# Cogito2012/OpenTAL

Measured on AMD Instinct MI355X. Metric: clips/sec training step, 256-frame THUMOS14 clips, higher is better.
Workload: dtype bf16

## Files before the change

### include/opental_hip.h

```cpp
#ifndef OPENTAL_HIP_H
#define OPENTAL_HIP_H

#include <stdint.h>
#include <stddef.h>

#ifdef __cplusplus
extern "C" {
#endif

#define OTAL_ABI_VERSION 26

#define OTAL_E_NULL      (-1)
#define OTAL_E_SHAPE     (-2)
#define OTAL_E_ODD_C     (-3)
#define OTAL_E_BATCH     (-4)
#define OTAL_E_DTYPE     (-5)
#define OTAL_E_LEVELS    (-6)
#define OTAL_E_UNSUPPORTED (-7)

#define OTAL_F32  0
#define OTAL_BF16 1
#define OTAL_F16  2
#define OTAL_F64  3

// ... 43 lines not shown
                         float* const* dw, int precision, void* ws, size_t ws_bytes, void* stream);

size_t otal_conv_prologue_bytes(const int* geom, const int64_t* strides, int mode, int precision);
size_t otal_conv_prologue_desc_bytes(void);
int otal_conv_prologue(const int* geom, const int64_t* strides, int mode, const float* w, int precision, void* region,
                       size_t region_bytes, void* host_desc, void* stream);
int otal_conv_prologue_batch(int n, const void* device_descs, const int* device_starts, int total_blocks, void* stream);

int otal_conv_defer_reduces(int on);
size_t otal_conv_deferred_end(void);
int otal_conv_deferred_count(void);
int otal_conv_flush_reduces(void* stream);

const char* otal_conv_last_kernel(void);

int otal_conv_pack_wt(const float* w, float* wt, int Cout, int Cin, int kvol, void* stream);

int otal_gn_relu_fwd(const float* x, const float* gamma, const float* beta, float* y, float* stats,
                     int B, int C, int T, int G, float eps, int relu, int nlev, const int* lev, void* stream);
int otal_gn_relu_bwd(const float* dy, int64_t dy_batch_stride, const float* x, const float* gamma, const float* beta,
                     const float* stats, float* dx, float* partial, int B, int C, int T, int G,
                     int relu, int nlev, const int* lev, void* stream);
int otal_gn_relu_fwd_pair(const float* const* x, const float* const* gamma, const float* const* beta, float* const* y,
                          float* const* stats, int B, int C, int T, int G, float eps, int relu, int nlev, const int* lev,
                          void* stream);
int otal_gn_relu_bwd_pair(const float* const* dy, const int64_t* dy_batch_stride, const float* const* x,
                          const float* const* gamma, const float* const* beta, const float* const* stats, float* const* dx,
                          float* const* partial, int B, int C, int T, int G, int relu, int nlev, const int* lev, void* stream);
int otal_sum_partials(int n_items, const float* const* partial, float* const* dst0, float* const* dst1,
                      float* const* dst2, const int* channels, const int* batches, void* stream);

const char* otal_layer_last_kernel(void);

int otal_maxpool3d_fwd(const int* geom, const int64_t* strides, const float* x, float* y,
                       unsigned char* argtap, void* stream);
int otal_maxpool3d_bwd(const int* geom, const int64_t* strides, const float* dy,
                       const unsigned char* argtap, float* dx, int accumulate,
                       const float* out_mask, const float* out_scale, void* stream);
size_t otal_maxpool3d_signbits_bytes(const int* geom, const int64_t* strides);
int otal_maxpool3d_fwd_signbits(const int* geom, const int64_t* strides, const float* x, float* y,
                                unsigned char* argtap, unsigned char* signbits, void* stream);
int otal_maxpool3d_bwd_signbits(const int* geom, const int64_t* strides, const float* dy, const unsigned char* argtap,
                                float* dx, int accumulate, const unsigned char* signbits, const float* out_scale,
                                void* stream);
int otal_maxpool3d_fwd_signbits_h(const int* geom, const int64_t* strides, const void* x_bf16, float* y,
                                  unsigned char* argtap, unsigned char* signbits, void* stream);
int otal_maxpool3d_bwd_signbits_h(const int* geom, const int64_t* strides, const float* dy, const unsigned char* argtap,
                                  void* dx_bf16, const unsigned char* signbits, const float* out_scale, void* stream);
int otal_maxpool3d_fwd_io(const int* geom, const int64_t* strides, const void* x, void* y, unsigned char* argtap,
                          unsigned char* signbits, int io, void* stream);
int otal_maxpool3d_bwd_io(const int* geom, const int64_t* strides, const void* dy, const unsigned char* argtap, void* dx,
                          int accumulate, const void* out_mask, const float* out_scale, const unsigned char* signbits, int io,
                          void* stream);
int otal_convert_storage(const void* src, int64_t src_bs, int64_t src_cs, void* dst, int64_t dst_bs, int64_t dst_cs,
                         int to_bf16, int B, int C, int P, void* stream);

int otal_head_outputs_fwd(int n_items, const int* channels, const int* modes, const float* const* raw, float* const* out,
                          float* const* unct, const float* scales, int B, int N, int nlev, const int* lev,
                          const float* level_strides, void* stream);
int otal_head_outputs_bwd(int n_items, const int* channels, const int* modes, const float* const* raw,
                          const float* const* out, const float* const* unct, const float* const* dout,
                          const float* const* dunct, float* const* draw, const float* scales, float* dscales, int B,
                          int N, int nlev, const int* lev, const float* level_strides, void* stream);

int otal_boundary_bce(const float* x, int64_t x_batch_stride, int64_t x_channel_stride, const float* mask,
                      int64_t mask_batch_stride, int64_t mask_row_stride, int mask_row0, int mask_step, float* terms,
                      float* dx, int B, int C, int T, void* stream);

int otal_boundary_finish(int n, const float* const* terms, const float* weights, const int* T, int B, float* out2, void* stream);
int otal_boundary_scale(int n, const float* const* dx, float* const* out, const float* weights, const int* C, const int* T,
                        int B, const float* g_start, const float* g_end, void* stream);

int otal_proposal_windows(const float* loc, float* seg, float* frame_seg, int B, int nlev,
                          const int* lev, float frame_num, void* stream);

int otal_decode_clips(const float* loc, const float* prop_loc, const float* priors, const float* conf,
                      const float* prop_conf, const float* center, const float* act, const float* prop_act,
                      const float* offsets, const float* fps, float* seg, float* score, float* unct,
                      float* actn, unsigned char* flag, int nclips, int A, int K, float clip_length,
                      float conf_thresh, void* stream);
int otal_decode_clips_ex(const float* loc, const float* prop_loc, const float* priors, const float* conf,
                         const float* prop_conf, const float* center, const float* act, const float* prop_act,
                         const float* offsets, const float* fps, float* seg, float* score, float* unct,
                         float* actn, unsigned char* flag, int nclips, int A, int K, float clip_length,
                         float conf_thresh, int score_fn, int first_class, void* stream);
int otal_softnms_classes(const float* seg, const float* score, const float* unct, const float* actn,
                         const unsigned char* flag, const int* clip_start, int nvideos, int max_clips,
                         int A, int K, float sigma, int top_k, float score_threshold, float* out,
                         int* counts, int* out_index, int out_cols, void* stream);
size_t otal_softnms_scratch_bytes(int total_clips, int max_clips, int A, int K);
int otal_softnms_classes_ws(const float* seg, const float* score, const float* unct, const float* actn,
                            const unsigned char* flag, const int* clip_start, int nvideos, int max_clips,
                            int A, int K, float sigma, int top_k, float score_threshold, float* out,
                            int* counts, int* out_index, int out_cols, void* scratch, size_t scratch_bytes,
                            int total_clips, void* stream);
int otal_detection_table(const float* rows, const int* counts, const double* durations, int V, int K, int top_k, int cols,
                         int drop_empty, int scoring, int* video, int* cls, double* seg, float* sup, double* known,
                         int* list_start, void* stream);

int otal_openmax_dist(const float* feat, int N, int rows_per_batch, int64_t sb, int64_t sr, int64_t sc, const float* mav,
                      int K, int D, const int* labels, float* dist, void* stream);
int otal_openmax_class_means(const float* feat, int N, int rows_per_batch, int64_t sb, int64_t sr, int64_t sc,
                             const int* labels, int K, int D, float* means, int* counts, void* stream);
int otal_openmax_probs(const float* logits, int64_t ldl, const float* feat, int N, int rows_per_batch, int64_t sb, int64_t sr,
                       int64_t sc, const float* mav, const float* wb, int K, int D, int R, float* probs, void* stream);
int otal_decode_clips_openmax(const float* loc, const float* prop_loc, const float* priors, const float* conf,
// ... 106 lines not shown
```

### opental_amd/common/i3d_backbone.py

```python
import torch
import torch.nn as nn
import torch.nn.functional as F
from torch.autograd import Function

from . import ops
from .layers import MaxPool3dSamePadding

ONE, THREE = (1, 1, 1), (3, 3, 3)
BN_EPS = 1e-3


class Unit3D(nn.Module):

    def __init__(self, in_channels, output_channels, kernel_shape=(1, 1, 1), stride=(1, 1, 1), padding=0,
                 activation_fn=F.relu, use_batch_norm=True, use_bias=False, padding_valid_spatial=False,
                 name='unit_3d'):
        super(Unit3D, self).__init__()
        if not use_batch_norm or use_bias or activation_fn is not F.relu or padding_valid_spatial or padding == -1:
            raise NotImplementedError("backbone Unit3D is conv(no bias) + BN + ReLU with SAME padding")
        self._output_channels = output_channels
        self._kernel_shape = tuple(kernel_shape)
        self._stride = tuple(stride)
        self.name = name
        self.conv3d = nn.Conv3d(in_channels, output_channels, self._kernel_shape, self._stride, padding=0, bias=False)
# ... 189 lines not shown
def _fused_affine(scale, shift, offs, w0):
    key = (scale.data_ptr(), shift.data_ptr(), scale._version, w0)
    hit = _FUSED_AFFINE.get(key)
    if hit is None:
        pick = lambda t, i: t[offs[i]:offs[i + 1]]
        hit = (torch.cat([pick(scale, w0 + 1), pick(scale, w0 + 3), pick(scale, w0)]),
               torch.cat([pick(shift, w0 + 1), pick(shift, w0 + 3), pick(shift, w0)]), scale, shift)
        if len(_FUSED_AFFINE) > 256:
            _FUSED_AFFINE.clear()
        _FUSED_AFFINE[key] = hit
    return hit[0], hit[1]


_HALF_OK = {}


def _pool_half_ok(shape, k, s):
    _, _, T, H, W = shape
    k, s = tuple(k), tuple(s)
    out_positions = -(-T // s[0]) * -(-H // s[1]) * -(-W // s[2])
    if out_positions % 8:
        return False
    if k[1:] == (3, 3) and s[1:] == (2, 2) and H % 2 == 0 and W % 4 == 0:
        return (k[0], s[0]) == (1, 1) or ((k[0], s[0]) == (3, 2) and T % 2 == 0)
    return k == THREE and s == ONE and H == W and H in (12, 6)


def _conv_half_ok(shape, cout, k, first=False):
    modes = (0, 2) if first else (0, 1, 2)
    return all(ops.half_storage_ok(m, tuple(shape), cout, k, ONE, both=True) for m in modes)


def _step_half_ok(step, shape, weights):
    key = (step[0], tuple(shape), step[1:-1] if step[0] != "conv" else (tuple(weights[step[1]].shape), step[2], step[3]), ops.HALF_CHAIN,
           int(ops.CONV_PRECISION), ops.HALF_STORAGE)
    hit = _HALF_OK.get(key)
    if hit is None:
        B, C, T, H, W = shape
        if not (ops.HALF_CHAIN and ops.HALF_STORAGE and int(ops.CONV_PRECISION) & 1):
            hit = False
        elif step[0] == "conv":
            hit = tuple(step[3]) == ONE and _conv_half_ok(shape, weights[step[1]].shape[0], tuple(step[2]))
        elif step[0] == "pool":
            hit = _pool_half_ok(shape, step[1], step[2])
        else:
            oc = step[2]
            hit = (_conv_half_ok(shape, oc[1] + oc[3] + oc[0], ONE) and _conv_half_ok((B, oc[1], T, H, W), oc[2], THREE)
                   and _conv_half_ok((B, oc[3], T, H, W), oc[4], THREE) and _pool_half_ok(shape, THREE, ONE)
                   and _conv_half_ok(shape, oc[5], ONE))
        if len(_HALF_OK) > 512:
            _HALF_OK.clear()
        _HALF_OK[key] = hit
    return hit


class I3DFeaturesFunction(Function):

    @staticmethod
    def forward(ctx, x, plan, endpoints, scale, shift, offs, *weights):
        x = x.contiguous()
        sc = lambda i: scale[offs[i]:offs[i + 1]]
        sh = lambda i: shift[offs[i]:offs[i + 1]]
        tape, found, half_grads = [], {}, {}
        cur = x
        cur_scale = None
        BF = torch.bfloat16
        need_grad = any(ctx.needs_input_grad)
        raw_out = {e[1:] for e in endpoints if e.startswith("=")}
        endpoints = tuple(e.lstrip("=") for e in endpoints)

        def leave_half():
            nonlocal cur
            cur32 = ops.convert_storage(cur, torch.float32)
            tape.append(("cvt", cur, cur32, cur_scale))
            cur = cur32

        for si, step in enumerate(plan):
            kind, name = step[0], step[-1]
            chain = cur.dtype == BF and _step_half_ok(step, cur.shape, weights)
            pool_io1 = (cur.dtype == BF and not chain and kind == "pool" and cur_scale is not None
                        and tuple(step[1]) == (1, 3, 3) and tuple(step[2]) == (1, 2, 2)
                        and cur.shape[3] % 2 == 0 and cur.shape[4] % 4 == 0)
            if cur.dtype == BF and not chain and not pool_io1:
                leave_half()
            if kind == "conv" and chain:
                _, wi, k, s, _ = step
                y = ops.conv_forward(cur, weights[wi], k, s, scale=sc(wi), shift=sh(wi), relu=True)
                tape.append(("conv", wi, k, s, cur, y, cur_scale, sc(wi)))
                cur, cur_scale = y, sc(wi)
            elif kind == "conv":
                _, wi, k, s, _ = step
                pooled_next = (name not in endpoints and si + 1 < len(plan) and plan[si + 1][0] == "pool"
                               and tuple(plan[si + 1][1]) == (1, 3, 3) and tuple(plan[si + 1][2]) == (1, 2, 2)
                               and ops.half_storage_ok(0, tuple(cur.shape), weights[wi].shape[0], k, s))
                grad_half = (pooled_next and si == 0 and not x.requires_grad
                             and ops.half_storage_ok(2, tuple(cur.shape), weights[wi].shape[0], k, s))
                half = pooled_next and (grad_half or (si > 0 and ops.HALF_ACT_DIRECT))
                if (not half and si == 0 and not x.requires_grad and ops.HALF_CHAIN and si + 1 < len(plan) and name not in endpoints
                        and ops.half_storage_ok(0, tuple(cur.shape), weights[wi].shape[0], k, s)
                        and ops.half_storage_ok(2, tuple(cur.shape), weights[wi].shape[0], k, s)):
                    half = True
                half_grads[si + 1] = grad_half
                y = ops.conv_forward(cur, weights[wi], k, s, scale=sc(wi), shift=sh(wi), relu=True, half_out=half)
                tape.append(("conv", wi, k, s, cur, y, cur_scale, sc(wi)))
                cur, cur_scale = y, sc(wi)
            elif kind == "pool":
# ... 38 lines not shown
                    ops.conv_forward(pm, weights[w0 + 5], ONE, ONE, scale=sc(w0 + 5), shift=sh(w0 + 5), relu=True,
                                     out=Y[:, c3:])
                out_scale = _cat_cached(_OUT_SCALE, scale, w0, [sc(w0), sc(w0 + 2), sc(w0 + 4), sc(w0 + 5)])
                tape.append(("mixed", w0, (c1, c2, c3), cur, h1, h2, pm, argm, Y, cur_scale, (wf, o1, o13), out_scale))
                cur, cur_scale = Y, out_scale
            if name in endpoints:
                if cur.dtype == BF and name not in raw_out:
                    ends = si + 1 == len(plan) or not _step_half_ok(plan[si + 1], cur.shape, weights)
                    if need_grad or ends:
                        leave_half()
                        found[name] = (cur, len(tape))
                    else:
                        found[name] = (ops.convert_storage(cur, torch.float32), len(tape))
                else:
                    found[name] = (cur, len(tape))
                hooks = ops.STEP.endpoint_hooks
                hook = hooks.get(name) if hooks else None
                if hook is not None:
                    hook(found[name][0])
        missing = [e for e in endpoints if e not in found]
        if missing:
            raise RuntimeError(f"unknown endpoints {missing}")
        ctx.tape = tape
        ctx.meta = (scale, offs, [found[e][1] for e in endpoints], len(weights), x.requires_grad)
        ctx.weights = weights
        ctx.outs = [found[e][0] for e in endpoints]
        return tuple(ctx.outs)

    @staticmethod
    def backward(ctx, *douts):
        tape, weights = ctx.tape, ctx.weights
        scale, offs, out_pos, nw, need_dx = ctx.meta
        sc = lambda i: scale[offs[i]:offs[i + 1]]
        dws = [None] * nw
        pending = {}
        for pos, g, z in zip(out_pos, douts, ctx.outs):
            if g is not None:
                pending.setdefault(pos, []).append((g, z, tape[pos - 1][-1]))
        zg = {}

        def out_grad_buffer(p, shape, like):
            if p >= 1 and tape[p - 1][0] == "mixed":
                o13 = tape[p - 1][10][2]
                B, ct, T, H, W = shape
                buf = torch.empty((B, o13 + ct, T, H, W), dtype=like.dtype, device=like.device)
                zg[p] = buf
                return buf[:, o13:]
            return torch.empty(tuple(shape), dtype=like.dtype, device=like.device)

        side = ops.side_wgrads(weights[0].device)
        in_slots = True
        dcur = None
        cloned = True
        mixed_pos = [p for p in range(1, len(tape) + 1) if tape[p - 1][0] == "mixed"]
        tail_below = min(mixed_pos) if mixed_pos and not need_dx else 0
        for pos in range(len(tape), 0, -1):
            if pos == tail_below - 1 and not any(pending.get(q) for q in range(1, pos + 1)):
                ops.late_mark([weights[st[1]] for st in tape[:pos] if st[0] == "conv"])
            for g, z, zs in pending.pop(pos, ()):
                ops.join_pending(g)
                dense = g.dim() == 5 and (g.shape[4] == 1 or g.stride(4) == 1) and (g.shape[3] == 1 or g.stride(3) == g.shape[4])
                if zs is not None and not dense:
                    g = g.contiguous()
                if dcur is None:
                    if zs is not None:
                        dcur = out_grad_buffer(pos, g.shape, g)
                        ops.masked_scale_copy(g, z, zs, dcur)
                    elif tape[pos - 1][0] == "mixed":
                        dcur = out_grad_buffer(pos, g.shape, g)
                        dcur.copy_(g)
                    else:
                        dcur = g.contiguous()
                        cloned = False
                elif zs is not None:
                    ops.masked_scale_copy(g, z, zs, dcur, accumulate=True)
                else:
                    if not cloned:
                        dcur, cloned = dcur.clone(), True
                    dcur.add_(g)
            if dcur is None:
                continue
            step = tape[pos - 1]
            first = pos == 1
            if step[0] == "cvt":
                _, xh, _, _ = step
                dcur = ops.convert_storage(dcur.contiguous(), xh.dtype, out=out_grad_buffer(pos - 1, xh.shape, xh))
            elif step[0] == "conv":
                _, wi, k, s, xin, y, in_scale, _ = step
                slot = ops.grad_slot(weights[wi])
                in_slots = in_slots and slot is not None
                if first and not need_dx:
                    side.issue()
                    dws[wi] = ops.conv_wgrad(xin, dcur, weights[wi].shape, k, s, out=slot)
                else:
                    dws[wi] = side.wgrad(xin, dcur, weights[wi].shape, k, s, out=slot)
                if first and not need_dx:
                    dcur = None
                else:
                    dcur = ops.conv_dgrad(dcur, weights[wi], xin.shape, k, s, out=out_grad_buffer(pos - 1, xin.shape, xin),
                                          out_mask=xin if in_scale is not None else None, out_scale=in_scale)
                side.flush()
                ops.grads_ready([(weights[wi], dws[wi])])
            elif step[0] == "pool":
                _, k, s, xin, (arg, bits, grad_half), in_scale, _ = step
                if dcur.dtype == torch.bfloat16:
                    masked = in_scale is not None and bits is not None
                    dcur = ops.maxpool3d_backward(dcur, arg, xin.shape, k, s, out=out_grad_buffer(pos - 1, xin.shape, xin),
                                                  out_scale=in_scale if masked else None, out_signbits=bits if masked else None)
                elif grad_half:
                    dcur = ops.maxpool3d_backward(dcur, arg, xin.shape, k, s, out_scale=in_scale, out_signbits=bits, half_out=True)
                else:
                    dcur = ops.maxpool3d_backward(dcur, arg, xin.shape, k, s, out=out_grad_buffer(pos - 1, xin.shape, dcur),
                                                  out_mask=xin if (in_scale is not None and bits is None) else None,
                                                  out_scale=in_scale, out_signbits=bits)
            else:
                _, w0, (c1, c2, c3), xin, h1, h2, pm, argm, Y, in_scale, (wf, o1, o13), _ = step
                Zg = zg.pop(pos)
                dY = Zg[:, o13:]
                dX = out_grad_buffer(pos - 1, xin.shape, xin)
                xm = xin if in_scale is not None else None
                sl = (slice(0, c1), slice(c1, c2), slice(c2, c3), slice(c3, Y.shape[1]))
                for a, b, hid, sli, dst in ((w0 + 1, w0 + 2, h1, sl[1], Zg[:, :o1]), (w0 + 3, w0 + 4, h2, sl[2], Zg[:, o1:o13])):
                    g = dY[:, sli]
                    slot = ops.grad_slot(weights[b])
                    in_slots = in_slots and slot is not None
                    dws[b] = side.wgrad(hid, g, weights[b].shape, THREE, ONE, out=slot)
                    ops.conv_dgrad(g, weights[b], hid.shape, THREE, ONE, out=dst, out_mask=hid, out_scale=sc(a))
                gf = Zg[:, :o13 + c1]
                slot = ops.grad_slot(wf)
                in_slots = in_slots and slot is not None
                dwf = side.wgrad(xin, gf, wf.shape, ONE, ONE, out=slot)
                dws[w0 + 1], dws[w0 + 3], dws[w0] = dwf[:o1], dwf[o1:o13], dwf[o13:]
                ops.conv_dgrad(gf, wf, xin.shape, ONE, ONE, out=dX, out_mask=xm, out_scale=in_scale)
                g3 = dY[:, sl[3]]
                slot = ops.grad_slot(weights[w0 + 5])
                in_slots = in_slots and slot is not None
                dws[w0 + 5] = side.wgrad(pm, g3, weights[w0 + 5].shape, ONE, ONE, out=slot)
                dpm = ops.conv_dgrad(g3, weights[w0 + 5], pm.shape, ONE, ONE)
                ops.maxpool3d_backward(dpm, argm, xin.shape, THREE, ONE, out=dX, accumulate=True,
                                       out_mask=xm, out_scale=in_scale)
                dcur = dX
                side.flush()
                ops.grads_ready([(weights[w0 + q], dws[w0 + q]) for q in range(6)])
        side.node_end(in_slots)
        ctx.tape = None
        ctx.outs = None
        dx = dcur if need_dx else None
        return (dx, None, None, None, None, None) + tuple(dws)
```

### opental_amd/common/ops.py

```python
import bisect
import ctypes
import os
import warnings

import torch

from .. import _lib as L
from .conv_geom import make_geom

_WORKSPACE = {}
WORKSPACE_BYTES = 192 << 20
WORKSPACE_TOTAL = 512 << 20

CONV_PROFILE = None

CONV_PRECISION = 0
HALF_STORAGE = os.environ.get("OTAL_HALF_STORAGE", "1") != "0"
HALF_ACT_DIRECT = os.environ.get("OTAL_HALF_ACT_DIRECT", "0") != "0"
HALF_CHAIN = os.environ.get("OTAL_HALF_CHAIN", "1") != "0"


def _prof_begin():
    if CONV_PROFILE is None:
        return None
    ev = torch.cuda.Event(enable_timing=True)
    ev.record()
    return ev


def _prof_end(ev, mode, g, problems=1):
    if ev is None:
        return
    end = torch.cuda.Event(enable_timing=True)
    end.record()
    B, Cin, Cout = g[0], g[1], g[2]
    flops = 2.0 * B * Cout * g[6] * g[7] * g[8] * Cin * g[9] * g[10] * g[11] * problems
    CONV_PROFILE.append((mode, flops, ev, end))


def workspace(device, side=False):
    key = (device.type, device.index, side)
    ws = _WORKSPACE.get(key)
    if ws is None:
        ws = torch.empty(WORKSPACE_TOTAL, dtype=torch.uint8, device=device)
        _WORKSPACE[key] = ws
    return ws


class StepState:
    def __init__(self):
        self.lanes = None
        self.slots = None
        self.ready = None
        self.defer_join = False
        self.pending_sums = None
        self.prologues = None
        self.late_weights = None
        self.endpoint_hooks = None
        self.early_results = {}
        self.pending_joins = {}
        self.defer = False
        self.defer_owner = None
        self.ws_cursor = [0, 0, 0, 0]
        self.ws_index = 0
        self.stream = None

    def begin_backward(self, slots, ready, early):
        if self.slots is not None:
            raise RuntimeError("a trainer's backward is already running in this process (one at a time)")
        self.slots, self.ready = slots, ready
        self.defer_join = early
        self.pending_sums = [] if early else None
# ... 1053 lines not shown
def maxpool3d_backward(dy, arg, x_shape, k, s, out=None, accumulate=False, out_mask=None, out_scale=None, out_signbits=None,
                       half_out=False):
    if dy.dtype == torch.bfloat16:
        if out is None:
            if accumulate:
                raise RuntimeError("accumulate needs an existing buffer")
            out = torch.empty(tuple(x_shape), dtype=torch.bfloat16, device=dy.device)
        g, outn = _pool_geom(out, k, s)
        _check(out, "dx", torch.bfloat16); _check(dy, "dy", torch.bfloat16)
        if tuple(dy.shape[2:]) != outn or not arg.is_contiguous():
            raise RuntimeError("maxpool3d_backward: shape mismatch")
        if out_mask is not None and (tuple(out_mask.shape) != tuple(out.shape) or out_mask.stride() != out.stride()
                                     or out_mask.dtype != torch.bfloat16):
            raise RuntimeError("out_mask must share dx's shape, layout and dtype")
        ga, sa = _geom_arrays(g, out, dy)
        L.check(L.lib().otal_maxpool3d_bwd_io(ga, sa, L.ptr(dy), L.ptr(arg), L.ptr(out), int(accumulate), _opt(out_mask),
                                              _opt(out_scale), _opt(out_signbits), 3 | (4 if out_mask is not None else 0), L.stream()),
                "otal_maxpool3d_bwd_io")
        return out
    if half_out:
        if accumulate or out_mask is not None or out_signbits is None or out is not None:
            raise RuntimeError("maxpool3d_backward(half_out): plain store with the sign-bit mask only")
        out = torch.empty(tuple(x_shape), dtype=torch.bfloat16, device=dy.device)
        g, outn = _pool_geom(out, k, s)
        _check(out, "dx", torch.bfloat16); _check(dy, "dy")
        if tuple(dy.shape[2:]) != outn or not arg.is_contiguous():
            raise RuntimeError("maxpool3d_backward: shape mismatch")
        ga, sa = _geom_arrays(g, out, dy)
        L.check(L.lib().otal_maxpool3d_bwd_signbits_h(ga, sa, L.ptr(dy), L.ptr(arg), L.ptr(out), L.ptr(out_signbits),
                                                      L.ptr(out_scale), L.stream()), "otal_maxpool3d_bwd_signbits_h")
        return out
    if out is None:
        if accumulate:
            raise RuntimeError("accumulate needs an existing buffer")
        out = torch.empty(tuple(x_shape), dtype=dy.dtype, device=dy.device)
    g, outn = _pool_geom(out, k, s)
    _check(out, "dx"); _check(dy, "dy")
    if tuple(dy.shape[2:]) != outn or not arg.is_contiguous():
        raise RuntimeError("maxpool3d_backward: shape mismatch")
    ga, sa = _geom_arrays(g, out, dy)
    if out_signbits is not None:
        if out.data_ptr() % 16 or dy.data_ptr() % 8:
            raise RuntimeError("maxpool3d_backward: the sign-bit path needs 16-byte aligned dx")
        L.check(L.lib().otal_maxpool3d_bwd_signbits(ga, sa, L.ptr(dy), L.ptr(arg), L.ptr(out), int(accumulate), L.ptr(out_signbits),
                                                    L.ptr(out_scale), L.stream()), "otal_maxpool3d_bwd_signbits")
        return out
    if out_mask is not None and (tuple(out_mask.shape) != tuple(out.shape) or out_mask.stride() != out.stride()):
        raise RuntimeError("out_mask must share dx's shape and layout")
    L.check(L.lib().otal_maxpool3d_bwd(ga, sa, L.ptr(dy), L.ptr(arg), L.ptr(out), int(accumulate),
                                       _opt(out_mask), _opt(out_scale), L.stream()), "otal_maxpool3d_bwd")
    return out


def convert_storage(src, dtype, out=None):
    s5 = _as5(src)
    if out is None:
        out = torch.empty(tuple(src.shape), dtype=dtype, device=src.device)
    o5 = _as5(out)
    if {src.dtype, out.dtype} != {torch.float32, torch.bfloat16} or tuple(o5.shape) != tuple(s5.shape):
        raise RuntimeError("convert_storage: float32 <-> bfloat16, same shape")
    _check(s5, "src", s5.dtype); _check(o5, "dst", o5.dtype)
    B, C, T, H, W = s5.shape
    if (T * H * W) % 8:
        out.copy_(src)
        return out
    (sb, sc), (db, dc) = _bs(s5), _bs(o5)
    L.check(L.lib().otal_convert_storage(L.ptr(s5), ctypes.c_int64(sb), ctypes.c_int64(sc), L.ptr(o5), ctypes.c_int64(db),
                                         ctypes.c_int64(dc), int(out.dtype == torch.bfloat16), B, C, T * H * W, L.stream()),
            "otal_convert_storage")
    return out


def proposal_windows(loc, levels, frame_num):
    L.require_device(loc)
    B, N, _ = loc.shape
    assert N == levels[-1]
    seg = torch.empty((B, N, 4), dtype=torch.float32, device=loc.device)
    fseg = torch.empty_like(seg)
    L.check(L.lib().otal_proposal_windows(L.ptr(loc), L.ptr(seg), L.ptr(fseg), B, len(levels) - 1,
                                          L.int_array(list(levels)), ctypes.c_float(frame_num), L.stream()),
            "otal_proposal_windows")
    return seg, fseg


def adam_flat(p, g, m, v, step, lr, beta1=0.9, beta2=0.999, eps=1e-8, weight_decay=0.0, grad_scale=1.0):
    L.require_device(p, g, m, v)
    L.check(L.lib().otal_adam_flat(L.ptr(p), L.ptr(g), L.ptr(m), L.ptr(v), ctypes.c_int64(p.numel()),
                                   ctypes.c_float(lr), ctypes.c_float(beta1), ctypes.c_float(beta2),
                                   ctypes.c_float(eps), ctypes.c_float(weight_decay), int(step),
                                   ctypes.c_float(grad_scale), L.stream()), "otal_adam_flat")


def adam_bias_corrections(step, beta1=0.9, beta2=0.999):
    import math
    import numpy as np
    b1, b2 = float(np.float32(beta1)), float(np.float32(beta2))
    return [float(np.float32(1.0 - math.pow(b1, step))), float(np.float32(math.sqrt(1.0 - math.pow(b2, step))))]


def adam_flat_dev(p, g, m, v, bias_corr, lr, beta1=0.9, beta2=0.999, eps=1e-8, weight_decay=0.0, grad_scale=1.0):
    L.require_device(p, g, m, v, bias_corr)
    L.check(L.lib().otal_adam_flat_dev(L.ptr(p), L.ptr(g), L.ptr(m), L.ptr(v), ctypes.c_int64(p.numel()),
                                       ctypes.c_float(lr), ctypes.c_float(beta1), ctypes.c_float(beta2),
                                       ctypes.c_float(eps), ctypes.c_float(weight_decay), L.ptr(bias_corr),
                                       ctypes.c_float(grad_scale), L.stream()), "otal_adam_flat_dev")

# ... 490 lines not shown
```

### opental_amd/csrc/pool3d.hip

```cpp
#include "common.h"
#include <cstdlib>

#include "pool_select.h"

namespace {

template <int KT, int KH, int KW, int ST, int SH, int SW>
struct PoolShape {
    __device__ __forceinline__ static int kt(const PoolGeom& g) { return KT ? KT : g.kt; }
    __device__ __forceinline__ static int kh(const PoolGeom& g) { return KT ? KH : g.kh; }
    __device__ __forceinline__ static int kw(const PoolGeom& g) { return KT ? KW : g.kw; }
    __device__ __forceinline__ static int st(const PoolGeom& g) { return KT ? ST : g.st; }
    __device__ __forceinline__ static int sh(const PoolGeom& g) { return KT ? SH : g.sh; }
    __device__ __forceinline__ static int sw(const PoolGeom& g) { return KT ? SW : g.sw; }
    static constexpr int UT = KT ? KT : 1, UH = KT ? KH : 1, UW = KT ? KW : 1;
    static constexpr int UCT = KT ? (KT + ST - 1) / ST : 1, UCH = KT ? (KH + SH - 1) / SH : 1, UCW = KT ? (KW + SW - 1) / SW : 1;
};

__device__ __forceinline__ float h2f_lo(unsigned w) { return __uint_as_float(w << 16); }
__device__ __forceinline__ float h2f_hi(unsigned w) { return __uint_as_float(w & 0xffff0000u); }
__device__ __forceinline__ unsigned f2h_pair_exact(float lo, float hi) {
    return (__float_as_uint(lo) >> 16) | (__float_as_uint(hi) & 0xffff0000u);
}
__device__ __forceinline__ unsigned f2h_pair_rne(float lo, float hi) {
// ... 192 lines not shown
    const int bc = blockIdx.y;
    const int b = bc / g.C, c = bc - b * g.C;
    const int to0 = blockIdx.x * TT;
    const int tt = min(TT, g.To - to0);
    const int TL = (tt - 1) * st + kt;
    const int PL = g.HL * g.WL;
    const float* xb = x + (int64_t)b * g.x_bs + (int64_t)c * g.x_cs;
    const int ti0 = to0 * st - g.pt;
    for (int i = threadIdx.x; i < TL * PL; i += 256) {
        const uint32_t tl = fd_div(g.fPL, (uint32_t)i);
        const uint32_t r = i - tl * PL;
        const uint32_t hl = fd_div(g.fWL, r);
        const int wl = (int)(r - hl * g.WL);
        const int ti = ti0 + (int)tl, hi = (int)hl - g.ph, wi = wl - g.pw;
        const bool in = (unsigned)ti < (unsigned)g.Ti && (unsigned)hi < (unsigned)g.Hi && (unsigned)wi < (unsigned)g.Wi;
        const int64_t off = in ? ((int64_t)ti * g.Hi + hi) * g.Wi + wi : 0;
        const float v = xb[off];
        sm[i] = in ? v : 0.f;
    }
    __syncthreads();
    const int Po = g.Ho * g.Wo;
    const int P = g.To * Po;
    for (int i = threadIdx.x; i < tt * Po; i += 256) {
        const uint32_t tq = fd_div(g.fPo, (uint32_t)i);
        const uint32_t r = i - tq * Po;
        const uint32_t ho = fd_div(g.fWo, r);
        const int wo = (int)(r - ho * g.Wo);
        const float* base = sm + ((int)tq * st * g.HL + (int)ho * sh) * g.WL + wo * sw;
        float best = 0.f;
        int win = 0;
        bool first = true;
#pragma unroll S::UT
        for (int dt = 0; dt < kt; ++dt)
#pragma unroll S::UH
            for (int dh = 0; dh < kh; ++dh)
#pragma unroll S::UW
                for (int dw = 0; dw < kw; ++dw) {
                    const float v = base[(dt * g.HL + dh) * g.WL + dw];
                    if (first || v > best || v != v) {
                        best = v;
                        win = (dt * kh + dh) * kw + dw;
                        first = false;
                    }
                }
        const int wdt = win / (kh * kw), wr = win - wdt * (kh * kw), wdh = wr / kw, wdw = wr - wdh * kw;
        const int ti = (to0 + (int)tq) * st - g.pt + wdt, hi = (int)ho * sh - g.ph + wdh, wi = wo * sw - g.pw + wdw;
        const bool in = (unsigned)ti < (unsigned)g.Ti && (unsigned)hi < (unsigned)g.Hi && (unsigned)wi < (unsigned)g.Wi;
        const int p = to0 * Po + i;
        y[(int64_t)b * g.y_bs + (int64_t)c * g.y_cs + p] = best;
        arg[(int64_t)bc * P + p] = (unsigned char)(in ? win : 255);
    }
}

template <int KT, int KH, int KW, int ST, int SH, int SW>
__global__ __launch_bounds__(256) void maxpool3d_bwd_lds_kernel(const float* __restrict__ dy,
                                                                const unsigned char* __restrict__ arg,
                                                                float* __restrict__ dx, PoolGeom g, int accumulate,
                                                                const float* __restrict__ emask,
                                                                const float* __restrict__ escale, int TI, int TLo_max) {
    using S = PoolShape<KT, KH, KW, ST, SH, SW>;
    extern __shared__ float sm[];
    const int kt = S::kt(g), kh = S::kh(g), kw = S::kw(g);
    const int st = S::st(g), sh = S::sh(g), sw = S::sw(g);
    constexpr int CT = KT ? (KT + ST - 1) / ST : 0, CH = KT ? (KH + SH - 1) / SH : 0, CW = KT ? (KW + SW - 1) / SW : 0;
    const int ct = KT ? CT : (kt + st - 1) / st, ch = KT ? CH : (kh + sh - 1) / sh, cw = KT ? CW : (kw + sw - 1) / sw;
    const int bc = blockIdx.y;
    const int b = bc / g.C, c = bc - b * g.C;
    const int ti0 = blockIdx.x * TI;
    const int tin = min(TI, g.Ti - ti0);
    const int toA = (ti0 + g.pt) / st - (ct - 1);
    const int toB = (ti0 + tin - 1 + g.pt) / st;
    const int TLo = toB - toA + 1;
    const int PLo = g.HLo * g.WLo;
    unsigned char* sa = reinterpret_cast<unsigned char*>(sm + TLo_max * PLo);
    const int Po = g.Ho * g.Wo;
    const float* dyb = dy + (int64_t)b * g.y_bs + (int64_t)c * g.y_cs;
    const unsigned char* ab = arg + (int64_t)bc * g.To * Po;
    for (int i = threadIdx.x; i < TLo * PLo; i += 256) {
        const uint32_t tl = fd_div(g.fPLo, (uint32_t)i);
        const uint32_t r = i - tl * PLo;
        const uint32_t hl = fd_div(g.fWLo, r);
        const int wl = (int)(r - hl * g.WLo);
        const int to = toA + (int)tl, ho = (int)hl + g.ho_min, wo = wl + g.wo_min;
        const bool in = (unsigned)to < (unsigned)g.To && (unsigned)ho < (unsigned)g.Ho && (unsigned)wo < (unsigned)g.Wo;
        const int o = in ? (to * g.Ho + ho) * g.Wo + wo : 0;
        const float d = dyb[o];
        const unsigned char a = ab[o];
        sm[i] = in ? d : 0.f;
        sa[i] = a;
    }
    __syncthreads();
    const int Pi = g.Hi * g.Wi;
    for (int i = threadIdx.x; i < tin * Pi; i += 256) {
        const uint32_t tq = fd_div(g.fPi, (uint32_t)i);
        const uint32_t r = i - tq * Pi;
        const uint32_t hi = fd_div(g.fWi, r);
        const int wi = (int)(r - hi * g.Wi);
        const int tn = ti0 + (int)tq + g.pt, hn = (int)hi + g.ph, wn = wi + g.pw;
        const int to0 = tn / st, ho0 = hn / sh, wo0 = wn / sw;
        float acc = 0.f;
#pragma unroll S::UCT
        for (int a_ = 0; a_ < ct; ++a_) {
            const int to = to0 - a_, dt = tn - to * st;
#pragma unroll S::UCH
            for (int b_ = 0; b_ < ch; ++b_) {
                const int ho = ho0 - b_, dh = hn - ho * sh;
#pragma unroll S::UCW
                for (int c_ = 0; c_ < cw; ++c_) {
                    const int wo = wo0 - c_, dw = wn - wo * sw;
                    const int idx = ((to - toA) * g.HLo + (ho - g.ho_min)) * g.WLo + (wo - g.wo_min);
                    const bool ok = dt < kt && dh < kh && dw < kw;
                    const float d = sm[idx];
                    const int a = sa[idx];
                    acc += (ok && a == (dt * kh + dh) * kw + dw) ? d : 0.f;
                }
            }
        }
        const int p = ti0 * Pi + i;
        const int64_t off = (int64_t)b * g.x_bs + (int64_t)c * g.x_cs + p;
        if (emask) acc = emask[off] > 0.f ? acc * escale[c] : 0.f;
        dx[off] = accumulate ? dx[off] + acc : acc;
    }
}

__device__ __forceinline__ void first_max3(float a, float b, float c, float& v, int& k) {
    v = a; k = 0;
    if (b > v || b != b) { v = b; k = 1; }
    if (c > v || c != c) { v = c; k = 2; }
}

template <int P>
__global__ __launch_bounds__(256) void maxpool333_sep_fwd_kernel(const float* __restrict__ x, float* __restrict__ y,
                                                                 unsigned char* __restrict__ arg, PoolGeom g, int TT, int vec) {
    extern __shared__ float sm[];
    constexpr int Q = P + 2, PL = Q * Q, PP = P * P, CR = Q * P;
    const int tid = threadIdx.x;
    const int bc = blockIdx.y;
    const int b = bc / g.C, c = bc - b * g.C;
    const int to0 = blockIdx.x * TT;
    const int tt = min(TT, g.To - to0);
    const int TL = tt + 2;
    float* xs = sm;
    float* rm = sm + (TT + 2) * PL;
    unsigned char* tw = reinterpret_cast<unsigned char*>(rm + (TT + 2) * CR);
    unsigned char* th = tw + (TT + 2) * CR;
    const float* xb = x + (int64_t)b * g.x_bs + (int64_t)c * g.x_cs;
    constexpr int VW = P % 4 == 0 ? 4 : (P % 2 == 0 ? 2 : 1);
    if (VW > 1 && vec) {
        for (int i = tid; i < TL * PL; i += 256) xs[i] = 0.f;
        __syncthreads();
        constexpr int NQ = P / VW;
        for (int i = tid; i < TL * P * NQ; i += 256) {
            const int tl = i / (P * NQ), r = i - tl * (P * NQ), hi = r / NQ, q = r - hi * NQ;
            const int ti = to0 - 1 + tl;
            if ((unsigned)ti >= (unsigned)g.Ti) continue;
            float* dst = xs + (tl * Q + hi + 1) * Q + q * VW + 1;
            if constexpr (VW == 4) {
                const float4 v = *reinterpret_cast<const float4*>(xb + (ti * P + hi) * P + q * 4);
                dst[0] = v.x; dst[1] = v.y; dst[2] = v.z; dst[3] = v.w;
            } else {
                const float2 v = *reinterpret_cast<const float2*>(xb + (ti * P + hi) * P + q * 2);
                dst[0] = v.x; dst[1] = v.y;
            }
        }
    } else {
        for (int i = tid; i < TL * PL; i += 256) {
            const int tl = i / PL, r = i - tl * PL, hl = r / Q, wl = r - hl * Q;
            const int ti = to0 - 1 + tl, hi = hl - 1, wi = wl - 1;
            const bool in = (unsigned)ti < (unsigned)g.Ti && (unsigned)hi < (unsigned)P && (unsigned)wi < (unsigned)P;
            const float v = xb[in ? (ti * P + hi) * P + wi : 0];
            xs[i] = in ? v : 0.f;
        }
    }
    __syncthreads();
// ... 875 lines not shown
        case PK_BWD_222: hipLaunchKernelGGL((maxpool3d_bwd_kernel<2, 2, 2, 2, 2, 2>), grid, block, c.lds, st_, dy, argtap, dx, g, acc, mask, scale); break;
        case PK_BWD_ANY: hipLaunchKernelGGL((maxpool3d_bwd_kernel<0, 0, 0, 0, 0, 0>), grid, block, c.lds, st_, dy, argtap, dx, g, acc, mask, scale); break;
        case PK_BWD_LDS_133: hipLaunchKernelGGL((maxpool3d_bwd_lds_kernel<1, 3, 3, 1, 2, 2>), grid, block, c.lds, st_, dy, argtap, dx, g, acc, mask, scale, c.planes, c.tlo_max); break;
        case PK_BWD_LDS_333S1: hipLaunchKernelGGL((maxpool3d_bwd_lds_kernel<3, 3, 3, 1, 1, 1>), grid, block, c.lds, st_, dy, argtap, dx, g, acc, mask, scale, c.planes, c.tlo_max); break;
        case PK_BWD_LDS_333S2: hipLaunchKernelGGL((maxpool3d_bwd_lds_kernel<3, 3, 3, 2, 2, 2>), grid, block, c.lds, st_, dy, argtap, dx, g, acc, mask, scale, c.planes, c.tlo_max); break;
        case PK_BWD_LDS_222: hipLaunchKernelGGL((maxpool3d_bwd_lds_kernel<2, 2, 2, 2, 2, 2>), grid, block, c.lds, st_, dy, argtap, dx, g, acc, mask, scale, c.planes, c.tlo_max); break;
        case PK_BWD_LDS_ANY: hipLaunchKernelGGL((maxpool3d_bwd_lds_kernel<0, 0, 0, 0, 0, 0>), grid, block, c.lds, st_, dy, argtap, dx, g, acc, mask, scale, c.planes, c.tlo_max); break;
        default: return OTAL_E_UNSUPPORTED;
    }
    return otal_layer_launched(pool_kernel_name(c.kernel));
}

extern "C" int otal_maxpool3d_fwd(const int* geom, const int64_t* strides, const float* x, float* y,
                                  unsigned char* argtap, void* stream) {
    return pool_fwd(geom, strides, x, y, argtap, nullptr, stream);
}
extern "C" int otal_maxpool3d_bwd(const int* geom, const int64_t* strides, const float* dy,
                                  const unsigned char* argtap, float* dx, int accumulate,
                                  const float* out_mask, const float* out_scale, void* stream) {
    return pool_bwd(geom, strides, dy, argtap, dx, accumulate, out_mask, out_scale, nullptr, stream);
}
extern "C" size_t otal_maxpool3d_signbits_bytes(const int* geom, const int64_t* strides) {
    if (!geom || !strides) return 0;
    PoolGeom g;
    if (fill(g, geom, strides)) return 0;
    if (!strided_k33_kind(g)) return 0;
    return (size_t)g.B * g.C * g.Ti * (g.Hi / 2) * (g.Wi / 4);
}
extern "C" int otal_maxpool3d_fwd_signbits(const int* geom, const int64_t* strides, const float* x, float* y,
                                           unsigned char* argtap, unsigned char* signbits, void* stream) {
    g_layer_kernel = "";
    if (!signbits) return OTAL_E_NULL;
    return pool_fwd(geom, strides, x, y, argtap, signbits, stream);
}
extern "C" int otal_maxpool3d_bwd_signbits(const int* geom, const int64_t* strides, const float* dy, const unsigned char* argtap,
                                           float* dx, int accumulate, const unsigned char* signbits, const float* out_scale,
                                           void* stream) {
    g_layer_kernel = "";
    if (!signbits || !out_scale) return OTAL_E_NULL;
    return pool_bwd(geom, strides, dy, argtap, dx, accumulate, nullptr, out_scale, signbits, stream);
}
extern "C" int otal_maxpool3d_fwd_signbits_h(const int* geom, const int64_t* strides, const void* x_bf16, float* y,
                                             unsigned char* argtap, unsigned char* signbits, void* stream) {
    g_layer_kernel = "";
    if (!signbits) return OTAL_E_NULL;
    return pool_fwd(geom, strides, static_cast<const float*>(x_bf16), y, argtap, signbits, stream, 1);
}
extern "C" int otal_maxpool3d_bwd_signbits_h(const int* geom, const int64_t* strides, const float* dy, const unsigned char* argtap,
                                             void* dx_bf16, const unsigned char* signbits, const float* out_scale, void* stream) {
    g_layer_kernel = "";
    if (!signbits || !out_scale) return OTAL_E_NULL;
    return pool_bwd(geom, strides, dy, argtap, static_cast<float*>(dx_bf16), 0, nullptr, out_scale, signbits, stream, 1);
}
extern "C" int otal_maxpool3d_fwd_io(const int* geom, const int64_t* strides, const void* x, void* y, unsigned char* argtap,
                                     unsigned char* signbits, int io, void* stream) {
    return pool_fwd(geom, strides, static_cast<const float*>(x), static_cast<float*>(y), argtap, signbits, stream, io);
}
extern "C" int otal_maxpool3d_bwd_io(const int* geom, const int64_t* strides, const void* dy, const unsigned char* argtap, void* dx,
                                     int accumulate, const void* out_mask, const float* out_scale, const unsigned char* signbits,
                                     int io, void* stream) {
    return pool_bwd(geom, strides, static_cast<const float*>(dy), argtap, static_cast<float*>(dx), accumulate,
                    static_cast<const float*>(out_mask), out_scale, signbits, stream, io);
}
```

Before: 1018.

## Fuse maxpool backward with bf16 convert, masked scale and residual add at seam

Adds a fused kernel for the backward pass at a pool step that directly follows an fp32-to-bf16 convert. It does the pool gradient gather, applies the ReLU mask and BN scale to both the pool gradient and a pending gradient, adds them, and writes bf16 straight into the upstream gradient buffer. The separate fp32 pool backward, the pending-gradient accumulation and the convert kernel are skipped. This removes several full-tensor fp32 read/write passes and kernel launches, in exchange for a narrower applicability check and fallbacks when the layout does not fit.

```diff
diff --git a/include/opental_hip.h b/include/opental_hip.h
--- a/include/opental_hip.h
+++ b/include/opental_hip.h
@@ -119,6 +119,9 @@
 int otal_maxpool3d_bwd_io(const int* geom, const int64_t* strides, const void* dy, const unsigned char* argtap, void* dx,
                           int accumulate, const void* out_mask, const float* out_scale, const unsigned char* signbits, int io,
                           void* stream);
+int otal_maxpool3d_bwd_seam(const int* geom, const int64_t* strides, const float* dy, const unsigned char* argtap,
+                            const void* mask_bf16, const int64_t* mask_strides, const float* out_scale,
+                            const float* add_src, const int64_t* add_strides, void* dx_bf16, void* stream);
 int otal_convert_storage(const void* src, int64_t src_bs, int64_t src_cs, void* dst, int64_t dst_bs, int64_t dst_cs,
                          int to_bf16, int B, int C, int P, void* stream);
 
diff --git a/opental_amd/common/i3d_backbone.py b/opental_amd/common/i3d_backbone.py
--- a/opental_amd/common/i3d_backbone.py
+++ b/opental_amd/common/i3d_backbone.py
@@ -265,6 +265,27 @@
             _HALF_OK.clear()
         _HALF_OK[key] = hit
     return hit
+
+
+def pool_seam_gradient(tape, pos, pending, zg, dcur):
+    if not ops.POOL_SEAM or pos < 2 or tape[pos - 1][0] != "pool" or tape[pos - 2][0] != "cvt":
+        return None
+    _, _, _, xin, (_, bits, grad_half), in_scale, _ = tape[pos - 1]
+    _, xh, x32, seam_scale = tape[pos - 2]
+    if xin is not x32 or in_scale is None or seam_scale is not in_scale or bits is not None or grad_half:
+        return None
+    if xh.dtype != torch.bfloat16 or dcur is None or dcur.dtype != torch.float32 or (pos - 2) in zg:
+        return None
+    waiting = pending.get(pos - 1) or ()
+    if len(waiting) != 1:
+        return None
+    g, z, zs = waiting[0]
+    if z is not x32 or zs is not in_scale or g.dtype != torch.float32 or g.dim() != 5 or tuple(g.shape) != tuple(xh.shape):
+        return None
+    dense = (g.shape[4] == 1 or g.stride(4) == 1) and (g.shape[3] == 1 or g.stride(3) == g.shape[4])
+    if not dense or (xh.shape[2] * xh.shape[3] * xh.shape[4]) % 8:
+        return None
+    return waiting[0]
 
 
 class I3DFeaturesFunction(Function):
@@ -409,6 +430,7 @@
         in_slots = True
         dcur = None
         cloned = True
+        seam_done = 0
         mixed_pos = [p for p in range(1, len(tape) + 1) if tape[p - 1][0] == "mixed"]
         tail_below = min(mixed_pos) if mixed_pos and not need_dx else 0
         for pos in range(len(tape), 0, -1):
@@ -439,7 +461,9 @@
                 continue
             step = tape[pos - 1]
             first = pos == 1
-            if step[0] == "cvt":
+            if step[0] == "cvt" and seam_done == pos:
+                pass
+            elif step[0] == "cvt":
                 _, xh, _, _ = step
                 dcur = ops.convert_storage(dcur.contiguous(), xh.dtype, out=out_grad_buffer(pos - 1, xh.shape, xh))
             elif step[0] == "conv":
@@ -460,6 +484,16 @@
                 ops.grads_ready([(weights[wi], dws[wi])])
             elif step[0] == "pool":
                 _, k, s, xin, (arg, bits, grad_half), in_scale, _ = step
+                seam = pool_seam_gradient(tape, pos, pending, zg, dcur)
+                if seam is not None:
+                    xh = tape[pos - 2][1]
+                    ops.join_pending(seam[0])
+                    dseam = out_grad_buffer(pos - 2, xh.shape, xh)
+                    if ops.maxpool3d_backward_seam(dcur, arg, k, s, xh, in_scale, seam[0], dseam):
+                        pending.pop(pos - 1)
+                        dcur, seam_done = dseam, pos - 1
+                        continue
+                    zg.pop(pos - 2, None)
                 if dcur.dtype == torch.bfloat16:
                     masked = in_scale is not None and bits is not None
                     dcur = ops.maxpool3d_backward(dcur, arg, xin.shape, k, s, out=out_grad_buffer(pos - 1, xin.shape, xin),
diff --git a/opental_amd/common/ops.py b/opental_amd/common/ops.py
--- a/opental_amd/common/ops.py
+++ b/opental_amd/common/ops.py
@@ -18,6 +18,7 @@
 HALF_STORAGE = os.environ.get("OTAL_HALF_STORAGE", "1") != "0"
 HALF_ACT_DIRECT = os.environ.get("OTAL_HALF_ACT_DIRECT", "0") != "0"
 HALF_CHAIN = os.environ.get("OTAL_HALF_CHAIN", "1") != "0"
+POOL_SEAM = True
 
 
 def _prof_begin():
@@ -1177,6 +1178,26 @@
     return out
 
 
+def maxpool3d_backward_seam(dy, arg, k, s, mask, scale, add_src, out):
+    B, C, T, H, W = out.shape
+    g, outn = _pool_geom(out, k, s)
+    _check(out, "dx", torch.bfloat16); _check(mask, "mask", torch.bfloat16); _check(dy, "dy")
+    if tuple(dy.shape) != (B, C) + outn or not arg.is_contiguous() or tuple(mask.shape) != tuple(out.shape):
+        raise RuntimeError("maxpool3d_backward_seam: shape mismatch")
+    if (not add_src.is_cuda or add_src.dtype != torch.float32 or tuple(add_src.shape) != tuple(out.shape)
+            or (W > 1 and add_src.stride(4) != 1) or (H > 1 and add_src.stride(3) != W)):
+        raise RuntimeError(f"maxpool3d_backward_seam: add_src must be a float32 GPU tensor of shape {tuple(out.shape)} with dense "
+                           f"H x W planes (strides {add_src.stride()})")
+    ga, sa = _geom_arrays(g, out, dy)
+    rc = L.lib().otal_maxpool3d_bwd_seam(ga, sa, L.ptr(dy), L.ptr(arg), L.ptr(mask), (ctypes.c_int64 * 2)(*_bs(mask)), L.ptr(scale),
+                                         L.ptr(add_src), (ctypes.c_int64 * 3)(add_src.stride(0), add_src.stride(1), add_src.stride(2)),
+                                         L.ptr(out), L.stream())
+    if rc == L.E_UNSUPPORTED:
+        return False
+    L.check(rc, "otal_maxpool3d_bwd_seam")
+    return True
+
+
 def convert_storage(src, dtype, out=None):
     s5 = _as5(src)
     if out is None:
diff --git a/opental_amd/csrc/pool3d.hip b/opental_amd/csrc/pool3d.hip
--- a/opental_amd/csrc/pool3d.hip
+++ b/opental_amd/csrc/pool3d.hip
@@ -268,6 +268,50 @@
     }
 }
 
+__device__ __forceinline__ void bwd_lds_stage(const float* __restrict__ dyb, const unsigned char* __restrict__ ab, const PoolGeom& g,
+                                              float* sm, unsigned char* sa, int toA, int TLo) {
+    const int PLo = g.HLo * g.WLo;
+    for (int i = threadIdx.x; i < TLo * PLo; i += 256) {
+        const uint32_t tl = fd_div(g.fPLo, (uint32_t)i);
+        const uint32_t r = i - tl * PLo;
+        const uint32_t hl = fd_div(g.fWLo, r);
+        const int wl = (int)(r - hl * g.WLo);
+        const int to = toA + (int)tl, ho = (int)hl + g.ho_min, wo = wl + g.wo_min;
+        const bool in = (unsigned)to < (unsigned)g.To && (unsigned)ho < (unsigned)g.Ho && (unsigned)wo < (unsigned)g.Wo;
+        const int o = in ? (to * g.Ho + ho) * g.Wo + wo : 0;
+        const float d = dyb[o];
+        const unsigned char a = ab[o];
+        sm[i] = in ? d : 0.f;
+        sa[i] = a;
+    }
+}
+template <class S>
+__device__ __forceinline__ float bwd_lds_gather(const float* sm, const unsigned char* sa, const PoolGeom& g, int toA, int tn, int hn, int wn,
+                                                int ct, int ch, int cw) {
+    const int kt = S::kt(g), kh = S::kh(g), kw = S::kw(g);
+    const int st = S::st(g), sh = S::sh(g), sw = S::sw(g);
+    const int to0 = tn / st, ho0 = hn / sh, wo0 = wn / sw;
+    float acc = 0.f;
+#pragma unroll S::UCT
+    for (int a_ = 0; a_ < ct; ++a_) {
+        const int to = to0 - a_, dt = tn - to * st;
+#pragma unroll S::UCH
+        for (int b_ = 0; b_ < ch; ++b_) {
+            const int ho = ho0 - b_, dh = hn - ho * sh;
+#pragma unroll S::UCW
+            for (int c_ = 0; c_ < cw; ++c_) {
+                const int wo = wo0 - c_, dw = wn - wo * sw;
+                const int idx = ((to - toA) * g.HLo + (ho - g.ho_min)) * g.WLo + (wo - g.wo_min);
+                const bool ok = dt < kt && dh < kh && dw < kw;
+                const float d = sm[idx];
+                const int a = sa[idx];
+                acc += (ok && a == (dt * kh + dh) * kw + dw) ? d : 0.f;
+            }
+        }
+    }
+    return acc;
+}
+
 template <int KT, int KH, int KW, int ST, int SH, int SW>
 __global__ __launch_bounds__(256) void maxpool3d_bwd_lds_kernel(const float* __restrict__ dy,
                                                                 const unsigned char* __restrict__ arg,
@@ -290,21 +334,7 @@
     const int PLo = g.HLo * g.WLo;
     unsigned char* sa = reinterpret_cast<unsigned char*>(sm + TLo_max * PLo);
     const int Po = g.Ho * g.Wo;
-    const float* dyb = dy + (int64_t)b * g.y_bs + (int64_t)c * g.y_cs;
-    const unsigned char* ab = arg + (int64_t)bc * g.To * Po;
-    for (int i = threadIdx.x; i < TLo * PLo; i += 256) {
-        const uint32_t tl = fd_div(g.fPLo, (uint32_t)i);
-        const uint32_t r = i - tl * PLo;
-        const uint32_t hl = fd_div(g.fWLo, r);
-        const int wl = (int)(r - hl * g.WLo);
-        const int to = toA + (int)tl, ho = (int)hl + g.ho_min, wo = wl + g.wo_min;
-        const bool in = (unsigned)to < (unsigned)g.To && (unsigned)ho < (unsigned)g.Ho && (unsigned)wo < (unsigned)g.Wo;
-        const int o = in ? (to * g.Ho + ho) * g.Wo + wo : 0;
-        const float d = dyb[o];
-        const unsigned char a = ab[o];
-        sm[i] = in ? d : 0.f;
-        sa[i] = a;
-    }
+    bwd_lds_stage(dy + (int64_t)b * g.y_bs + (int64_t)c * g.y_cs, arg + (int64_t)bc * g.To * Po, g, sm, sa, toA, TLo);
     __syncthreads();
     const int Pi = g.Hi * g.Wi;
     for (int i = threadIdx.x; i < tin * Pi; i += 256) {
@@ -312,30 +342,89 @@
         const uint32_t r = i - tq * Pi;
         const uint32_t hi = fd_div(g.fWi, r);
         const int wi = (int)(r - hi * g.Wi);
-        const int tn = ti0 + (int)tq + g.pt, hn = (int)hi + g.ph, wn = wi + g.pw;
-        const int to0 = tn / st, ho0 = hn / sh, wo0 = wn / sw;
-        float acc = 0.f;
-#pragma unroll S::UCT
-        for (int a_ = 0; a_ < ct; ++a_) {
-            const int to = to0 - a_, dt = tn - to * st;
-#pragma unroll S::UCH
-            for (int b_ = 0; b_ < ch; ++b_) {
-                const int ho = ho0 - b_, dh = hn - ho * sh;
-#pragma unroll S::UCW
-                for (int c_ = 0; c_ < cw; ++c_) {
-                    const int wo = wo0 - c_, dw = wn - wo * sw;
-                    const int idx = ((to - toA) * g.HLo + (ho - g.ho_min)) * g.WLo + (wo - g.wo_min);
-                    const bool ok = dt < kt && dh < kh && dw < kw;
-                    const float d = sm[idx];
-                    const int a = sa[idx];
-                    acc += (ok && a == (dt * kh + dh) * kw + dw) ? d : 0.f;
-                }
-            }
-        }
+        float acc = bwd_lds_gather<S>(sm, sa, g, toA, ti0 + (int)tq + g.pt, (int)hi + g.ph, wi + g.pw, ct, ch, cw);
         const int p = ti0 * Pi + i;
         const int64_t off = (int64_t)b * g.x_bs + (int64_t)c * g.x_cs + p;
         if (emask) acc = emask[off] > 0.f ? acc * escale[c] : 0.f;
         dx[off] = accumulate ? dx[off] + acc : acc;
+    }
+}
+
+struct AddStrides { int64_t b, c, t; };
+template <int KT, int KH, int KW, int ST, int SH, int SW, bool AV>
+__global__ __launch_bounds__(256) void maxpool3d_bwd_seam_kernel(const float* __restrict__ dy, const unsigned char* __restrict__ arg,
+                                                                 unsigned short* __restrict__ dx, PoolGeom g,
+                                                                 const unsigned short* __restrict__ mask, int64_t m_bs, int64_t m_cs,
+                                                                 const float* __restrict__ escale, const float* __restrict__ add,
+                                                                 AddStrides as, int TI, int TLo_max) {
+    using S = PoolShape<KT, KH, KW, ST, SH, SW>;
+    extern __shared__ float sm[];
+    const int kt = S::kt(g), kh = S::kh(g), kw = S::kw(g);
+    const int st = S::st(g), sh = S::sh(g), sw = S::sw(g);
+    constexpr int CT = KT ? (KT + ST - 1) / ST : 0, CH = KT ? (KH + SH - 1) / SH : 0, CW = KT ? (KW + SW - 1) / SW : 0;
+    const int ct = KT ? CT : (kt + st - 1) / st, ch = KT ? CH : (kh + sh - 1) / sh, cw = KT ? CW : (kw + sw - 1) / sw;
+    const int bc = blockIdx.y;
+    const int b = bc / g.C, c = bc - b * g.C;
+    const int ti0 = blockIdx.x * TI;
+    const int tin = min(TI, g.Ti - ti0);
+    const int toA = (ti0 + g.pt) / st - (ct - 1);
+    const int toB = (ti0 + tin - 1 + g.pt) / st;
+    const int TLo = toB - toA + 1;
+    const int PLo = g.HLo * g.WLo;
+    unsigned char* sa = reinterpret_cast<unsigned char*>(sm + TLo_max * PLo);
+    const int Po = g.Ho * g.Wo;
+    bwd_lds_stage(dy + (int64_t)b * g.y_bs + (int64_t)c * g.y_cs, arg + (int64_t)bc * g.To * Po, g, sm, sa, toA, TLo);
+    __syncthreads();
+    const int Pi = g.Hi * g.Wi;
+    const int lo = ti0 * Pi, hi = lo + tin * Pi;
+    const unsigned short* mb = mask + (int64_t)b * m_bs + (int64_t)c * m_cs;
+    unsigned short* db = dx + (int64_t)b * g.x_bs + (int64_t)c * g.x_cs;
+    const float* addb = add + (int64_t)b * as.b + (int64_t)c * as.c;
+    const float esc = escale[c];
+    auto pool_term = [&](int e, int64_t& aoff) {
+        const uint32_t t = fd_div(g.fPi, (uint32_t)e);
+        const uint32_t r = e - t * Pi;
+        const uint32_t h = fd_div(g.fWi, r);
+        const int w = (int)(r - h * g.Wi);
+        aoff = (int64_t)t * as.t + r;
+        return bwd_lds_gather<S>(sm, sa, g, toA, (int)t + g.pt, (int)h + g.ph, w + g.pw, ct, ch, cw);
+    };
+    auto combine = [&](float p, float m, float a) {
+        const float first = m > 0.f ? p * esc : 0.f;
+        const float second = m > 0.f ? a * esc : 0.f;
+        return first + second;
+    };
+    for (int k = (lo >> 3) + threadIdx.x; k < ((hi + 7) >> 3); k += 256) {
+        const int e0 = k * 8;
+        if (e0 >= lo && e0 + 8 <= hi) {
+            const uint4 mw = *reinterpret_cast<const uint4*>(mb + e0);
+            const unsigned mws[4] = {mw.x, mw.y, mw.z, mw.w};
+            float p[8], a[8], o[8];
+            int64_t aoff[8];
+#pragma unroll
+            for (int j = 0; j < 8; ++j) p[j] = pool_term(e0 + j, aoff[j]);
+            if constexpr (AV) {
+#pragma unroll
+                for (int q = 0; q < 2; ++q) {
+                    const float4 v = *reinterpret_cast<const float4*>(addb + aoff[4 * q]);
+                    a[4 * q] = v.x; a[4 * q + 1] = v.y; a[4 * q + 2] = v.z; a[4 * q + 3] = v.w;
+                }
+            } else {
+#pragma unroll
+                for (int j = 0; j < 8; ++j) a[j] = addb[aoff[j]];
+            }
+#pragma unroll
+            for (int j = 0; j < 8; ++j) o[j] = combine(p[j], (j & 1) ? h2f_hi(mws[j >> 1]) : h2f_lo(mws[j >> 1]), a[j]);
+            *reinterpret_cast<uint4*>(db + e0) = make_uint4(f2h_pair_rne(o[0], o[1]), f2h_pair_rne(o[2], o[3]),
+                                                            f2h_pair_rne(o[4], o[5]), f2h_pair_rne(o[6], o[7]));
+        } else {
+            for (int e = max(e0, lo); e < min(e0 + 8, hi); ++e) {
+                int64_t aoff;
+                const float p = pool_term(e, aoff);
+                const float o = combine(p, h2f_lo(mb[e]), addb[aoff]);
+                db[e] = (unsigned short)(f2h_pair_rne(o, 0.f) & 0xffffu);
+            }
+        }
     }
 }
 
@@ -1317,6 +1406,38 @@
     if (!signbits || !out_scale) return OTAL_E_NULL;
     return pool_bwd(geom, strides, dy, argtap, static_cast<float*>(dx_bf16), 0, nullptr, out_scale, signbits, stream, 1);
 }
+extern "C" int otal_maxpool3d_bwd_seam(const int* geom, const int64_t* strides, const float* dy, const unsigned char* argtap,
+                                       const void* mask_bf16, const int64_t* mask_strides, const float* out_scale,
+                                       const float* add_src, const int64_t* add_strides, void* dx_bf16, void* stream) {
+    g_layer_kernel = "";
+    if (!geom || !strides || !dy || !argtap || !mask_bf16 || !mask_strides || !out_scale || !add_src || !add_strides || !dx_bf16) return OTAL_E_NULL;
+    PoolQuery q = {};
+    q.dir = POOL_BWD; q.has_mask = 1; q.has_scale = 1;
+    q.x = (uintptr_t)dx_bf16; q.y = (uintptr_t)dy; q.argtap = (uintptr_t)argtap; q.mask = (uintptr_t)mask_bf16;
+    q.geom_rc = fill(q.g, geom, strides);
+    const PoolChoice c = pool_choose(q);
+    if (c.rc) return c.rc;
+    const PoolGeom& g = q.g;
+    if (c.kernel < PK_BWD_LDS_133 || c.kernel > PK_BWD_LDS_ANY) return OTAL_E_UNSUPPORTED;
+    const bool generic = c.kernel != PK_BWD_LDS_222;
+    const int64_t P = (int64_t)g.Ti * g.Hi * g.Wi;
+    const int64_t m_bs = mask_strides[0], m_cs = mask_strides[1];
+    if (P % 8 || g.x_bs % 8 || g.x_cs % 8 || m_bs % 8 || m_cs % 8 ||
+        ((reinterpret_cast<uintptr_t>(dx_bf16) | reinterpret_cast<uintptr_t>(mask_bf16)) & 15)) return OTAL_E_UNSUPPORTED;
+    const AddStrides as{add_strides[0], add_strides[1], add_strides[2]};
+    const bool av = (g.Hi * g.Wi) % 4 == 0 && as.b % 4 == 0 && as.c % 4 == 0 && as.t % 4 == 0 && (reinterpret_cast<uintptr_t>(add_src) & 15) == 0;
+    const dim3 grid(c.gx, c.gy), block(256);
+    hipStream_t st_ = (hipStream_t)stream;
+    unsigned short* dx = static_cast<unsigned short*>(dx_bf16);
+    const unsigned short* mk = static_cast<const unsigned short*>(mask_bf16);
+#define OTAL_SEAM_LAUNCH(...) hipLaunchKernelGGL((maxpool3d_bwd_seam_kernel<__VA_ARGS__>), grid, block, c.lds, st_, dy, argtap, dx, g, mk, m_bs, m_cs, \
+                                                 out_scale, add_src, as, c.planes, c.tlo_max)
+    if (generic) { if (av) OTAL_SEAM_LAUNCH(0, 0, 0, 0, 0, 0, true); else OTAL_SEAM_LAUNCH(0, 0, 0, 0, 0, 0, false); }
+    else { if (av) OTAL_SEAM_LAUNCH(2, 2, 2, 2, 2, 2, true); else OTAL_SEAM_LAUNCH(2, 2, 2, 2, 2, 2, false); }
+#undef OTAL_SEAM_LAUNCH
+    return otal_layer_launched(generic ? "maxpool3d_bwd_seam<generic>" : "maxpool3d_bwd_seam<222/222>");
+}
+
 extern "C" int otal_maxpool3d_fwd_io(const int* geom, const int64_t* strides, const void* x, void* y, unsigned char* argtap,
                                      unsigned char* signbits, int io, void* stream) {
     return pool_fwd(geom, strides, static_cast<const float*>(x), static_cast<float*>(y), argtap, signbits, stream, io);
```

Result: no change. 1022 (median of 2 runs) (+0.4%).
